# megvii-research/Far3D

Measured on AMD Instinct MI355X. Metric: samples/sec (7-cam frame) end-to-end @ VoV-99 640x960, higher is better.
Workload: dtype bf16x3; 1 GPU; BASELINE configs[1]: 7 cameras 3x640x960, VoV-99, A=1544 queries (644 learned + 644 adaptive + 256 propagated), 2312 self-attn keys, 6 decoder layers, streaming memory on, ego motion on; proposals=topk, fused_rows=True, parallelism=single GPU, weights=seeded random (far3d_amd.weights.init_state_dict, seed 0)

## Files before the change

### far3d_amd/csrc/conv_ws.hip

```cpp
#include "conv_ws.hpp"
#include "far3d_hip.h"

#ifdef FAR3D_PROFILING
std::atomic<int> g_ws_ablate{0};
extern "C" int far3d_conv_ws_set_ablate(int mask) { g_ws_ablate.store(mask); return 0; }
#endif

#define WS_CAPS_SINGLE(id, ...) case id: return Conv3x3WsShape<__VA_ARGS__>::caps;
#define WS_CAPS_GROUPED(id, ...)                                                   \
  case id: return Conv3x3WsShape<__VA_ARGS__>::caps | FAR3D_TILE_HAS_GROUP;        \
  case id + 100: return Conv3x3WsShape<__VA_ARGS__>::caps | FAR3D_TILE_GROUPED;
#define WS_CAPS_GROUPED_PLAIN(id, ...) WS_CAPS_GROUPED(id, __VA_ARGS__)
#define WS_CAPS(a, id, mark, ...) WS_CAPS_##mark(id, __VA_ARGS__)
#define WS_GROUP_SINGLE(id, ...)
#define WS_GROUP_GROUPED(id, ...) case id + 100: return launch_conv3x3_ws_grouped<true, __VA_ARGS__>(P, G, st);
#define WS_GROUP_GROUPED_PLAIN(id, ...) case id + 100: return launch_conv3x3_ws_grouped<false, __VA_ARGS__>(P, G, st);
#define WS_GROUP(a, id, mark, ...) WS_GROUP_##mark(id, __VA_ARGS__)
#define WS_LAUNCH(a, id, mark, ...) case id: return launch_conv3x3_ws<__VA_ARGS__>(P, st);

int far3d_ws_tile_caps(int tile) {
  switch (tile) {
    FAR3D_TILES_WS_CONV3(WS_CAPS, )
    FAR3D_TILES_WS_GEMM(TILE_CAPS, Gemm1x1WsShape)
    default: return -1;
  }
}

int far3d_conv_ws_launch(const IgemmParams& P, int tile, hipStream_t st) {
  switch (tile) {
    FAR3D_TILES_WS_CONV3(WS_LAUNCH, )
    default: break;
  }
  far3d_set_error("far3d_conv2d_nhwc: unknown wave-specialised tile %d", tile);
  return FAR3D_ERR_ARG;
}

extern "C" int far3d_ws_deal(int n_full, int n_light, int grid, int wg, int k) {
  if (n_full < 0 || n_light < 0 || grid < 1 || wg < 0 || wg >= grid) return -1;
  return ws_deal_item(n_full, n_light, grid, wg, k);
}

int far3d_gemm_ws_launch(const IgemmParams& P, int tile, hipStream_t st) {
  switch (tile) {
    FAR3D_TILES_WS_GEMM(TILE_LAUNCH, launch_gemm1x1_ws)
    default: break;
  }
  far3d_set_error("far3d_conv2d_nhwc: unknown wave-specialised GEMM tile %d", tile);
  return FAR3D_ERR_ARG;
}

static int far3d_conv_ws_grouped_launch(const IgemmParams& P, const WsGroup& G, int tile, hipStream_t st) {
  switch (tile) {
    FAR3D_TILES_WS_CONV3(WS_GROUP, )
    default: break;
  }
  far3d_set_error("far3d_conv2d_nhwc_grouped: unknown grouped tile %d", tile);
  return FAR3D_ERR_ARG;
}

extern "C" int far3d_conv2d_nhwc_grouped(const far3d_conv_problem* probs, int n, int tile, void* stream) {
  FAR3D_CHECK_ARG(probs && n >= 1 && n <= FAR3D_WS_GROUP_MAX, "far3d_conv2d_nhwc_grouped: %d problems (1..%d)", n, FAR3D_WS_GROUP_MAX);
  const int caps = far3d_ws_tile_caps(tile);
  FAR3D_CHECK_ARG(caps >= 0 && (caps & FAR3D_TILE_GROUPED), "far3d_conv2d_nhwc_grouped: tile %d is not a grouped tile (conv_tiles.hpp: 100 + a marked 4xx id)", tile);
  auto aligned = [](const void* p, long a) { return ((uintptr_t)p % a) == 0; };
  WsGroup G;
  memset(&G, 0, sizeof(G));
  G.n = n;
  const int Cin = probs[0].Cin;
  for (int i = 0; i < n; ++i) {
    const far3d_conv_problem& c = probs[i];
    FAR3D_CHECK_ARG(c.Cin == Cin, "far3d_conv2d_nhwc_grouped: problem %d has Cin %d, problem 0 has %d (one Cin per launch)", i, c.Cin, Cin);
    FAR3D_CHECK_ARG(c.x && c.w && c.y && c.N > 0 && c.H > 0 && c.W > 0 && c.Cout > 0 && Cin > 0 && Cin % 32 == 0 && c.Cout % 32 == 0 &&
                    c.act >= 0 && c.act <= 2 && c.ldx >= 2 * Cin && c.ldy >= 2 * c.Cout &&
                    aligned(c.x, 16) && aligned(c.y, 16) && c.ldx % 8 == 0 && c.ldy % 8 == 0 && c.x_img_stride % 8 == 0 && c.y_img_stride % 8 == 0 &&
                    (long)c.N * c.H * c.W < (1L << 31) - 4096 && (long)c.H * c.W * c.ldx * 2 < 0x7fffffffL,
                    "far3d_conv2d_nhwc_grouped: problem %d: needs pair-stored maps in and out, Cin and Cout multiples of 32, 16-byte aligned rows "
                    "(N=%d H=%d W=%d Cin=%d Cout=%d ldx=%d ldy=%d act=%d)", i, c.N, c.H, c.W, c.Cin, c.Cout, c.ldx, c.ldy, c.act);
    FAR3D_CHECK_ARG(!c.y2 || (c.y2_scale && c.y2_shift && aligned(c.y2, 16) && aligned(c.y2_scale, 16) && aligned(c.y2_shift, 16) &&
                              c.ldy2 >= c.Cout && c.ldy2 % 4 == 0 && c.y2_img_stride % 4 == 0),
                    "far3d_conv2d_nhwc_grouped: problem %d: the second output is fp32 with 16-byte aligned rows, scale and shift", i);
    WsProblem& q = G.p[i];
// ... 20 lines not shown
```

### far3d_amd/csrc/conv_ws.hpp

```cpp
#pragma once
#include "igemm_kernels.hpp"
#include <type_traits>

__device__ __forceinline__ __amdgpu_buffer_rsrc_t uniform_rsrc(const void* p, long nbytes) {
  const unsigned long long a = (unsigned long long)(uintptr_t)p;
  const unsigned lo = __builtin_amdgcn_readfirstlane((unsigned)a), hi = __builtin_amdgcn_readfirstlane((unsigned)(a >> 32));
  const int nb = __builtin_amdgcn_readfirstlane((int)(nbytes < 0x7fffffffL ? nbytes : 0x7fffffffL));
  return __builtin_amdgcn_make_buffer_rsrc((void*)(uintptr_t)(((unsigned long long)hi << 32) | lo), 0, nb, 0x00020000);
}

__device__ __forceinline__ void wait_vmcnt_dyn(int n) {
#define FAR3D_WVC(k) case k: wait_vmcnt<k>(); break;
  switch (n) {
    FAR3D_WVC(0) FAR3D_WVC(1) FAR3D_WVC(2) FAR3D_WVC(3) FAR3D_WVC(4) FAR3D_WVC(5) FAR3D_WVC(6) FAR3D_WVC(7) FAR3D_WVC(8)
    FAR3D_WVC(9) FAR3D_WVC(10) FAR3D_WVC(11) FAR3D_WVC(12) FAR3D_WVC(13) FAR3D_WVC(14) FAR3D_WVC(15) FAR3D_WVC(16)
    FAR3D_WVC(17) FAR3D_WVC(18) FAR3D_WVC(19) FAR3D_WVC(20) FAR3D_WVC(21) FAR3D_WVC(22) FAR3D_WVC(23) FAR3D_WVC(24)
    FAR3D_WVC(25) FAR3D_WVC(26) FAR3D_WVC(27) FAR3D_WVC(28) FAR3D_WVC(29) FAR3D_WVC(30) FAR3D_WVC(31) FAR3D_WVC(32)
    FAR3D_WVC(33) FAR3D_WVC(34) FAR3D_WVC(35) FAR3D_WVC(36) FAR3D_WVC(37) FAR3D_WVC(38) FAR3D_WVC(39) FAR3D_WVC(40)
    FAR3D_WVC(41) FAR3D_WVC(42) FAR3D_WVC(43) FAR3D_WVC(44) FAR3D_WVC(45) FAR3D_WVC(46) FAR3D_WVC(47)
    default: wait_vmcnt<48>(); break;
  }
#undef FAR3D_WVC
}

// ... 594 lines not shown
            const float4 bq = b4[q >> 1][q & 1];
            pacc[i][j][4 * q + 0] = acc[i][j][4 * q + 0] + bq.x; pacc[i][j][4 * q + 1] = acc[i][j][4 * q + 1] + bq.y;
            pacc[i][j][4 * q + 2] = acc[i][j][4 * q + 2] + bq.z; pacc[i][j][4 * q + 3] = acc[i][j][4 * q + 3] + bq.w;
          }
      }
      pd_n = n; pd_y0 = y0; pd_x0 = x0; pd_m0 = m0; pd_prob = prob;
    } else {
#pragma unroll
      for (int j = 0; j < WN; ++j)
#pragma unroll
        for (int i = 0; i < WM; ++i)
#pragma unroll
          for (int qp = 0; qp < 2; ++qp) {
            float4 b4[2];
            epi_bias(i, qp, m0, prob, b4);
            epi_slice(std::false_type{}, acc, i, j, qp, n, y0, x0, m0, prob, &b4);
          }
    }
#ifdef FAR3D_PROFILING
    if (pf_on) pf_epi += __builtin_amdgcn_s_memtime() - pf_e0;
#endif
  }
#ifdef FAR3D_PROFILING
  if (P.prof && t == 0) {
    P.prof[(long)blockIdx.x * 16 + 3] = (unsigned long long)__builtin_amdgcn_s_memtime();
    P.prof[(long)blockIdx.x * 16 + 7] = (unsigned long long)__builtin_amdgcn_s_memrealtime();
    P.prof[(long)blockIdx.x * 16 + 5] = (unsigned long long)total_steps;
    P.prof[(long)blockIdx.x * 16 + 8] = pf_wait; P.prof[(long)blockIdx.x * 16 + 9] = pf_body; P.prof[(long)blockIdx.x * 16 + 10] = pf_epi;
  }
#endif
#endif
}

template <int WGM, int WGN, int WM, int WN, int NP, int NSW, int GRP, bool SUMS>
__global__ __launch_bounds__(64 * (WGM * WGN + NP)) void gemm1x1_ws_kernel(IgemmParams P, int npt, int nct, int ablate) {
#if defined(__HIP_DEVICE_COMPILE__)
  constexpr int NWC = WGM * WGN;
  constexpr int BM = 32 * WGM * WM, BP = 32 * WGN * WN;
  constexpr int GA = BM / 16, GB = BP / 16, SLOTS = GA + GB;
  static_assert(SLOTS % NP == 0, "every producer issues the same number of pieces per step (counted vmcnt)");
  constexpr int SPW = SLOTS / NP;
  constexpr int SUB = (BM + BP) * 64, STAGE = 2 * SUB;
  static_assert(NSW % GRP == 0 && NSW / GRP >= 2, "ring = at least two hand-over groups");
  constexpr int NG = NSW / GRP;
  extern __shared__ __attribute__((aligned(1024))) unsigned char smem[];
  const int t = threadIdx.x, lane = t & 63, wv = __builtin_amdgcn_readfirstlane(t >> 6);
  constexpr int SUMB = NSW * STAGE;
  static_assert(SUMB + 4 * BM * 8 <= 163840, "LDS budget");
  [[maybe_unused]] long long* const lsum = reinterpret_cast<long long*>(smem + SUMB);
  constexpr bool do_sums = SUMS;
  if (do_sums) {
    for (int i = threadIdx.x; i < 4 * BM; i += 64 * (NWC + NP)) lsum[i] = 0;
    __syncthreads();
  }
  const int HoWo = P.Ho * P.Wo;
  const long Npix = (long)P.N * HoWo;
  const int nsteps = P.cin_pad / 32;
  const int Ktot = P.cin_pad * 2;
  const int xcd = (int)blockIdx.x & 7, slot0 = (int)blockIdx.x >> 3, dslot = (int)gridDim.x >> 3;
  const int vslots = ((npt - xcd + 7) >> 3) * nct;
  const int my_items = vslots > slot0 ? (vslots - slot0 + dslot - 1) / dslot : 0;
  const int total_steps = my_items * nsteps;
  const int total_groups = (total_steps + GRP - 1) / GRP;
  auto decode = [&](int k, int& p0, int& m0) __attribute__((always_inline)) {
    const int slot = slot0 + k * dslot;
    const int ct = slot % nct, pt = (slot / nct) * 8 + xcd;
    p0 = __builtin_amdgcn_readfirstlane(pt * BP); m0 = __builtin_amdgcn_readfirstlane(ct * BM);
  };

  if (wv >= NWC) {
    const int pw = wv - NWC;
    const int rg = lane >> 2, pc = lane & 3;
    const int lc = pc ^ ((rg >> 2) & 3);
    constexpr unsigned OOB = 0x80000000u;
    const long x_bytes = ((long)(P.N - 1) * P.x_img_stride + (long)HoWo * P.ldx) * 2;
    unsigned voff[SPW];
    int sdst[SPW];
    bool isw[SPW];
#pragma unroll
    for (int i = 0; i < SPW; ++i) {
      const int q = pw + NP * i;
      isw[i] = q < GA;
      const int g = isw[i] ? q : q - GA;
      sdst[i] = (isw[i] ? 0 : BM * 64) + g * 1024;
      voff[i] = isw[i] ? (unsigned)(((g * 16 + rg) * Ktot + lc * 8) * 2) : 0u;
    }
    const bf16_t* w_base = nullptr;
    long w_bytes = 0;
    int cur_tile = 0, cur_step = 0, cur_stage = 0, left = total_steps;
    auto set_tile = [&](int k) __attribute__((always_inline)) {
      int p0, m0;
      decode(k, p0, m0);
      w_base = reinterpret_cast<const bf16_t*>(P.w) + (long)m0 * Ktot;
      w_bytes = w_tile_bytes(BM, m0, P.Cout, Ktot);
#pragma unroll
      for (int i = 0; i < SPW; ++i) {
        if (!isw[i]) {
          const int g = pw + NP * i - GA;
          const long p = (long)p0 + g * 16 + rg;
          if (p < Npix) {
            int n, rem;
            pix_split(p, HoWo, n, rem);
            voff[i] = (unsigned)(((long)n * P.x_img_stride + (long)rem * P.ldx + lc * 8) * 2);
          } else {
            voff[i] = OOB;
          }
        }
      }
    };
    auto next = [&]() __attribute__((always_inline)) {
      if (!(ablate & 1)) {
        const __amdgpu_buffer_rsrc_t rs_w = uniform_rsrc(w_base, w_bytes);
        const __amdgpu_buffer_rsrc_t rs_x = uniform_rsrc(P.x, x_bytes);
        const int sbase = __builtin_amdgcn_readfirstlane(cur_stage * STAGE);
        const int kb = __builtin_amdgcn_readfirstlane(cur_step * 128);
#pragma unroll
        for (int i = 0; i < SPW; ++i) {
#pragma unroll
          for (int pl = 0; pl < 2; ++pl) {
            if (isw[i])
              __builtin_amdgcn_raw_ptr_buffer_load_lds(rs_w, (lds_void_t*)(smem + sbase + pl * SUB + sdst[i]), 16, voff[i], kb + pl * 64, 0, 0);
            else
              __builtin_amdgcn_raw_ptr_buffer_load_lds(rs_x, (lds_void_t*)(smem + sbase + pl * SUB + sdst[i]), 16, voff[i], kb + pl * 64, 0, 0);
          }
        }
      }
      --left;
      cur_stage = cur_stage == NSW - 1 ? 0 : cur_stage + 1;
      if (++cur_step == nsteps) { cur_step = 0; ++cur_tile; if (left > 0) set_tile(cur_tile); }
    };
    if (my_items > 0) set_tile(0);
#pragma unroll
    for (int i = 0; i < (NG - 1) * GRP; ++i)
      if (left > 0) next();
    for (int g = 0; g < total_groups; ++g) {
      int later = total_steps - (g + 1) * GRP;
      later = later < 0 ? 0 : (later > (NG - 2) * GRP ? (NG - 2) * GRP : later);
      if (ablate & 1) wait_vmcnt<0>(); else wait_vmcnt_dyn(later * SPW * 2);
      __builtin_amdgcn_s_barrier();
      asm volatile("" ::: "memory");
#pragma unroll
      for (int i = 0; i < GRP; ++i)
        if (left > 0) next();
    }
    if (do_sums) __builtin_amdgcn_s_barrier();
    return;
  }

  const int wm = wv / WGN, wn = wv % WGN, l31 = lane & 31, hi = lane >> 5;
  int aaddr[WM], baddr[WN];
#pragma unroll
  for (int i = 0; i < WM; ++i) {
    const int r = (wm * WM + i) * 32 + l31;
    aaddr[i] = r * 64 + ((hi ^ ((r >> 2) & 3)) << 4);
  }
#pragma unroll
  for (int j = 0; j < WN; ++j) {
    const int r = (wn * WN + j) * 32 + l31;
    baddr[j] = BM * 64 + r * 64 + ((hi ^ ((r >> 2) & 3)) << 4);
  }
  f32x16_t acc[WM][WN];
  u32x4_t fa[2][2][WM], fb[2][2][WN];
  auto load_a = [&](int set, int soff, int kk) __attribute__((always_inline)) {
    const int x32 = kk * 32;
#pragma unroll
    for (int pl = 0; pl < 2; ++pl)
#pragma unroll
      for (int i = 0; i < WM; ++i) fa[set][pl][i] = *reinterpret_cast<const u32x4_t*>(smem + pl * SUB + ((aaddr[i] ^ x32) + soff));
  };
  auto load_b = [&](int set, int soff, int kk) __attribute__((always_inline)) {
    const int x32 = kk * 32;
#pragma unroll
    for (int pl = 0; pl < 2; ++pl)
#pragma unroll
      for (int j = 0; j < WN; ++j) fb[set][pl][j] = *reinterpret_cast<const u32x4_t*>(smem + pl * SUB + ((baddr[j] ^ x32) + soff));
  };
  auto mma_term = [&](int set, int term) __attribute__((always_inline)) {
    const int pa = term == 0 ? 1 : 0, pb = term == 1 ? 1 : 0;
#pragma unroll
    for (int i = 0; i < WM; ++i)
#pragma unroll
      for (int j = 0; j < WN; ++j) mma<bf16_t>(acc[i][j], fa[set][pa][i], fb[set][pb][j]);
  };
  int soff = 0, gs = 0;
  [[maybe_unused]] int flush_tile = 0, gcount = 0;
  auto flush = [&](int T) __attribute__((always_inline)) {
    int fp0, fm0;
    decode(T, fp0, fm0);
    const int fcam0 = (int)((long)fp0 / P.sums_hw);
    long long* src = lsum + (T & 1) * 2 * BM;
    for (int i = wv * 64 + lane; i < 2 * BM; i += 64 * NWC) {
      const int sl = i / BM, chn = i - sl * BM, cam = fcam0 + sl;
      const long long v = src[i];
      if (v != 0) {
        src[i] = 0;
        if (cam < P.N && fm0 + chn < P.Cout)
          atomicAdd(reinterpret_cast<unsigned long long*>(P.chan_sums + (long)cam * P.Cout + fm0 + chn), (unsigned long long)v);
      }
    }
  };
  for (int k = 0; k < my_items; ++k) {
    int p0, m0;
    decode(k, p0, m0);
#pragma unroll
    for (int i = 0; i < WM; ++i)
#pragma unroll
      for (int j = 0; j < WN; ++j)
#pragma unroll
        for (int r = 0; r < 16; ++r) acc[i][j][r] = 0.f;
    for (int s = 0; s < nsteps; ++s) {
      const int stage = soff;
      if (gs == 0) {
        __builtin_amdgcn_s_waitcnt(0xc07f);
        __builtin_amdgcn_s_barrier();
        asm volatile("" ::: "memory");
        __builtin_amdgcn_sched_barrier(0);
        if constexpr (do_sums) {
          while (flush_tile < k && ((flush_tile + 1) * nsteps - 1) / GRP < gcount) { flush(flush_tile); ++flush_tile; }
          ++gcount;
        }
      }
      gs = gs == GRP - 1 ? 0 : gs + 1;
      if (ablate & 2) { soff = soff == (NSW - 1) * STAGE ? 0 : soff + STAGE; continue; }
      load_a(0, stage, 0); load_b(0, stage, 0);
      __builtin_amdgcn_sched_barrier(0);
      if (s > 0) { mma_term(1, 0); mma_term(1, 1); mma_term(1, 2); }
      __builtin_amdgcn_sched_barrier(0);
      load_a(1, stage, 1);
      __builtin_amdgcn_sched_barrier(0);
      mma_term(0, 0);
      __builtin_amdgcn_sched_barrier(0);
      load_b(1, stage, 1);
      __builtin_amdgcn_sched_barrier(0);
      mma_term(0, 1);
      mma_term(0, 2);
      __builtin_amdgcn_sched_barrier(0);
      soff = soff == (NSW - 1) * STAGE ? 0 : soff + STAGE;
    }
    if (!(ablate & 2)) { mma_term(1, 0); mma_term(1, 1); mma_term(1, 2); }
    __builtin_amdgcn_sched_barrier(0);

    {
      unsigned char* yb = reinterpret_cast<unsigned char*>(P.y);
      const int cam0 = do_sums ? (int)((long)p0 / P.sums_hw) : 0;
      const long bnd = (long)(cam0 + 1) * P.sums_hw;
      const bool two = do_sums && (long)p0 + BP > bnd;
      long pix_b[WN];
      bool okj[WN], secj[WN];
#pragma unroll
      for (int j = 0; j < WN; ++j) {
        const long p = (long)p0 + (wn * WN + j) * 32 + l31;
        okj[j] = p < Npix;
        secj[j] = p >= bnd;
        pix_b[j] = 0;
        if (okj[j]) {
          int n, rem;
          pix_split(p, HoWo, n, rem);
          pix_b[j] = ((long)n * P.y_img_stride + (long)rem * P.ldy) * 2;
        }
      }
      auto stored = [&](int i, int j, int q, int cb, uint2& h, uint2& l) __attribute__((always_inline)) {
        float4 b4 = make_float4(0.f, 0.f, 0.f, 0.f);
        if (P.bias) b4 = *reinterpret_cast<const float4*>(P.bias + cb + 8 * q + 4 * hi);
        float v[4];
#pragma unroll
        for (int e = 0; e < 4; ++e) v[e] = acc[i][j][4 * q + e];
        v[0] += b4.x; v[1] += b4.y; v[2] += b4.z; v[3] += b4.w;
        if (P.act == ACT_RELU) {
#pragma unroll
          for (int e = 0; e < 4; ++e) v[e] = fmaxf(v[e], 0.f);
        } else if (P.act == ACT_SWISH) {
#pragma unroll
          for (int e = 0; e < 4; ++e) v[e] = v[e] * (1.f / (1.f + expf(-v[e])));
        }
        split4f(v[0], v[1], v[2], v[3], h, l);
      };
      auto quantise = [&](const uint2& h, const uint2& l, int q, int (&qs)[16], float& mx) __attribute__((always_inline)) {
        const unsigned w4[4] = {h.x, h.y, l.x, l.y};
#pragma unroll
        for (int e = 0; e < 2; ++e) {
          const float h0 = __uint_as_float(w4[e] << 16), h1 = __uint_as_float(w4[e] & 0xffff0000u);
          const float l0 = __uint_as_float(w4[2 + e] << 16), l1 = __uint_as_float(w4[2 + e] & 0xffff0000u);
          mx = fmaxf(mx, fmaxf(fabsf(h0), fabsf(h1)));
          qs[4 * q + 2 * e] += __float2int_rn(h0 * (float)(1 << FAR3D_SUMS_FRAC_BITS)) + __float2int_rn(l0 * (float)(1 << FAR3D_SUMS_FRAC_BITS));
          qs[4 * q + 2 * e + 1] += __float2int_rn(h1 * (float)(1 << FAR3D_SUMS_FRAC_BITS)) + __float2int_rn(l1 * (float)(1 << FAR3D_SUMS_FRAC_BITS));
        }
      };
      auto half_sum = [&](int x) __attribute__((always_inline)) -> int {
        x += __builtin_amdgcn_update_dpp(0, x, 0x128, 0xf, 0xf, true);
        x += __builtin_amdgcn_update_dpp(0, x, 0x124, 0xf, 0xf, true);
        x += __builtin_amdgcn_update_dpp(0, x, 0x122, 0xf, 0xf, true);
        x += __builtin_amdgcn_update_dpp(0, x, 0x121, 0xf, 0xf, true);
        typedef unsigned u2_t __attribute__((ext_vector_type(2)));
        const u2_t r = __builtin_amdgcn_permlane16_swap((unsigned)x, (unsigned)x, false, false);
        const unsigned rx = r.x, ry = r.y;
        return (int)(rx + ry);
      };
      auto reduce_add = [&](const int (&qs)[16], float mx, int sl, int cb) __attribute__((always_inline)) {
        const bool wide = WN > 2 || __any(mx >= (float)(1 << (24 - FAR3D_SUMS_FRAC_BITS)));
        long long* dst = lsum + ((k & 1) * 2 + sl) * BM + (cb - m0) + 4 * hi;
#pragma unroll
        for (int r = 0; r < 16; ++r) {
          long long tot;
          if (!wide) {
            tot = (long long)half_sum(qs[r]);
          } else {
            const int lo16 = qs[r] & 0xffff, hi16 = qs[r] >> 16;
            tot = (long long)half_sum(hi16) * 65536ll + (long long)half_sum(lo16);
          }
          if (l31 == 0 && tot != 0) atomicAdd(reinterpret_cast<unsigned long long*>(dst + 8 * (r >> 2) + (r & 3)), (unsigned long long)tot);
        }
      };
      auto channel_block = [&](auto ic) __attribute__((always_inline)) {
        constexpr int i = decltype(ic)::value;
        const int cb = m0 + (wm * WM + i) * 32;
        if (cb >= P.Cout) return;
        int qs[16];
        float mx = 0.f;
#pragma unroll
        for (int r = 0; r < 16; ++r) qs[r] = 0;
#pragma unroll
        for (int j = 0; j < WN; ++j) {
#pragma unroll
          for (int qp = 0; qp < 2; ++qp) {
            uint2 h[2], l[2];
#pragma unroll
            for (int u = 0; u < 2; ++u) {
              stored(i, j, 2 * qp + u, cb, h[u], l[u]);
              if (do_sums && okj[j] && !secj[j]) quantise(h[u], l[u], 2 * qp + u, qs, mx);
            }
            u32x4_t oh, ol;
            {
              const auto sx = __builtin_amdgcn_permlane32_swap(h[0].x, h[1].x, false, false);
              const auto sy = __builtin_amdgcn_permlane32_swap(h[0].y, h[1].y, false, false);
              oh = u32x4_t{sx[0], sy[0], sx[1], sy[1]};
            }
            {
              const auto sx = __builtin_amdgcn_permlane32_swap(l[0].x, l[1].x, false, false);
              const auto sy = __builtin_amdgcn_permlane32_swap(l[0].y, l[1].y, false, false);
              ol = u32x4_t{sx[0], sy[0], sx[1], sy[1]};
            }
            if (okj[j]) {
              unsigned char* d = yb + pix_b[j] + (long)(cb >> 5) * 128 + (2 * qp + hi) * 16;
              *reinterpret_cast<u32x4_t*>(d) = oh;
              *reinterpret_cast<u32x4_t*>(d + 64) = ol;
            }
          }
        }
        if constexpr (do_sums) {
          auto exact_add = [&](int sl) __attribute__((always_inline)) {
            long long* dst = lsum + ((k & 1) * 2 + sl) * BM + (cb - m0) + 4 * hi;
#pragma unroll
            for (int q = 0; q < 4; ++q) {
              long long x[4] = {0, 0, 0, 0};
#pragma unroll
// ... 14 lines not shown
#pragma unroll
              for (int e = 0; e < 4; ++e) {
                const long long v = x[e];
                const long long tot = (long long)half_sum((int)(v & 0xffff)) + ((long long)half_sum((int)((v >> 16) & 0xffff)) << 16) +
                                      ((long long)half_sum((int)((v >> 32) & 0xffff)) << 32) + ((long long)half_sum((int)(v >> 48)) << 48);
                if (l31 == 0 && tot != 0) atomicAdd(reinterpret_cast<unsigned long long*>(dst + 8 * q + e), (unsigned long long)tot);
              }
            }
          };
          const bool huge = __any(mx >= 2048.f);
          if (huge) exact_add(0); else reduce_add(qs, mx, 0, cb);
          if (two) {
            float mx1 = 0.f;
#pragma unroll
            for (int r = 0; r < 16; ++r) qs[r] = 0;
#pragma unroll
            for (int j = 0; j < WN; ++j)
#pragma unroll
              for (int q = 0; q < 4; ++q) {
                uint2 h, l;
                stored(i, j, q, cb, h, l);
                if (okj[j] && secj[j]) quantise(h, l, q, qs, mx1);
              }
            if (__any(mx1 >= 2048.f)) exact_add(1); else reduce_add(qs, mx1, 1, cb);
          }
        }
      };
      static_assert(WM <= 4, "channel blocks per consumer");
      channel_block(std::integral_constant<int, 0>{});
      if constexpr (WM > 1) channel_block(std::integral_constant<int, 1>{});
      if constexpr (WM > 2) channel_block(std::integral_constant<int, 2>{});
      if constexpr (WM > 3) channel_block(std::integral_constant<int, 3>{});
    }
  }
  if constexpr (do_sums) {
    __builtin_amdgcn_s_waitcnt(0xc07f);
    __builtin_amdgcn_s_barrier();
    asm volatile("" ::: "memory");
    while (flush_tile < my_items) { flush(flush_tile); ++flush_tile; }
  }
#endif
}

static int ws_cu_count() {
  static std::atomic<int> n_cu{0};
  int cus = n_cu.load(std::memory_order_relaxed);
  if (cus == 0) {
    int dev = 0;
    if (hipGetDevice(&dev) != hipSuccess) dev = 0;
    if (hipDeviceGetAttribute(&cus, hipDeviceAttributeMultiprocessorCount, dev) != hipSuccess || cus <= 0) cus = 256;
    n_cu.store(cus, std::memory_order_relaxed);
  }
  return cus;
}
constexpr int ws_wg_per_cu(size_t lds, int threads) { return lds <= 81920 && threads <= 1024 ? 2 : 1; }

template <int WGM, int WGN, int WM, int WN, int NP, int NSW, int GRP>
struct Gemm1x1WsShape {
  static constexpr int BM = 32 * WGM * WM, BP = 32 * WGN * WN, THREADS = 64 * (WGM * WGN + NP);
  static constexpr size_t lds = (size_t)NSW * 2 * (BM + BP) * 64 + 4 * BM * 8;
  static constexpr int wg_per_cu = ws_wg_per_cu(lds, THREADS);
  static constexpr int caps = tile_caps(FAR3D_TILE_1X1, FAR3D_TILE_PAIR, BP, FAR3D_TILE_LDS_DMA | FAR3D_TILE_PERSISTENT | FAR3D_TILE_SUMS);
};

template <int WGM, int WGN, int WM, int WN, int NP, int NSW, int GRP>
static int launch_gemm1x1_ws(const IgemmParams& P, hipStream_t st) {
  using S = Gemm1x1WsShape<WGM, WGN, WM, WN, NP, NSW, GRP>;
  constexpr int BM = S::BM, BP = S::BP;
  constexpr size_t lds = S::lds;
  static_assert(lds <= 163840, "LDS budget");
  const long Npix = (long)P.N * P.Ho * P.Wo;
  const int npt = (int)((Npix + BP - 1) / BP), nct = (P.Cout + BM - 1) / BM;
  static std::atomic<unsigned long long> lds_ok_s{0};
  const long items = (long)((npt + 7) / 8 * 8) * nct;
  long grid = (long)ws_cu_count() * S::wg_per_cu;
  grid = (grid + 7) / 8 * 8;
  if (items < grid) grid = items;
  static std::atomic<unsigned long long> lds_ok{0};
  if constexpr (lds > 65536)
    if (const int rc = far3d_allow_lds(P.chan_sums ? reinterpret_cast<const void*>(&gemm1x1_ws_kernel<WGM, WGN, WM, WN, NP, NSW, GRP, true>)
                                                   : reinterpret_cast<const void*>(&gemm1x1_ws_kernel<WGM, WGN, WM, WN, NP, NSW, GRP, false>),
                                       (int)lds, P.chan_sums ? lds_ok_s : lds_ok, "far3d_conv2d_nhwc")) return rc;
  if (P.chan_sums) {
    if (P.sums_hw < BP || P.cin_pad / 32 < 2 * GRP) {
      far3d_set_error("far3d_conv2d_nhwc: channel sums on this wave-specialised GEMM tile need Ho*Wo (%d) >= %d pixels and Cin >= %d", P.sums_hw, BP, 64 * GRP);
      return FAR3D_ERR_ARG;
    }
    hipLaunchKernelGGL((gemm1x1_ws_kernel<WGM, WGN, WM, WN, NP, NSW, GRP, true>), dim3((unsigned)grid), dim3(S::THREADS), lds, st, P, npt, nct, FAR3D_WS_ABLATE_ARG);
  } else {
    hipLaunchKernelGGL((gemm1x1_ws_kernel<WGM, WGN, WM, WN, NP, NSW, GRP, false>), dim3((unsigned)grid), dim3(S::THREADS), lds, st, P, npt, nct, FAR3D_WS_ABLATE_ARG);
  }
  return 0;
}

template <int WGM, int WGN, int WM, int WN, int NP, bool PAIR, bool DBUF, int NSW = 3, bool FLAGS = false, int GRP = 1, bool DEFER = false>
struct Conv3x3WsShape {
  static constexpr int BM = 32 * WGM * WM, TH = WGN * WN, PLD = PAIR ? 2 : 1, THREADS = 64 * (WGM * WGN + NP);
  static constexpr int PG = (34 * (TH + 2) + 15) / 16;
  static constexpr size_t lds = (size_t)NSW * PLD * BM * 64 + (size_t)2 * PLD * PG * 1024 + (FLAGS ? 128 : 0);
  static constexpr int wg_per_cu = ws_wg_per_cu(lds, THREADS);
  static constexpr int caps = tile_caps(FAR3D_TILE_3X3, PAIR ? FAR3D_TILE_PAIR : FAR3D_TILE_BF16, 32 * TH, FAR3D_TILE_LDS_DMA | FAR3D_TILE_PERSISTENT);
};

template <bool DEFER_OK, int WGM, int WGN, int WM, int WN, int NP, bool PAIR, bool DBUF, int NSW = 3, bool FLAGS = false, int GRP = 1, bool DEFER = false, class GT>
static int launch_conv3x3_ws_items(const IgemmParams& P, hipStream_t st, int tiles_x, int tiles_y, int n_mt, int n_items, const GT& G, const char* who) {
  using S = Conv3x3WsShape<WGM, WGN, WM, WN, NP, PAIR, DBUF, NSW, FLAGS, GRP, DEFER>;
  static_assert(S::lds <= 163840, "LDS budget");
  const int resident = ws_cu_count() * S::wg_per_cu;
  const int grid = n_items < resident ? n_items : resident;
  static std::atomic<unsigned long long> lds_ok{0};
  if constexpr (S::lds > 65536)
    if (const int rc = far3d_allow_lds(reinterpret_cast<const void*>(&conv3x3_ws_kernel<WGM, WGN, WM, WN, NP, PAIR, DBUF, NSW, FLAGS, GRP, GT, DEFER && DEFER_OK>), (int)S::lds, lds_ok, who)) return rc;
  hipLaunchKernelGGL((conv3x3_ws_kernel<WGM, WGN, WM, WN, NP, PAIR, DBUF, NSW, FLAGS, GRP, GT, DEFER && DEFER_OK>), dim3((unsigned)grid), dim3(S::THREADS), S::lds, st, P, tiles_x, tiles_y,
                     n_mt, n_items, FAR3D_WS_ABLATE_ARG, G);
  return 0;
}

template <int WGM, int WGN, int WM, int WN, int NP, bool PAIR, bool DBUF, auto... MORE>
static int launch_conv3x3_ws(const IgemmParams& P, hipStream_t st) {
  using S = Conv3x3WsShape<WGM, WGN, WM, WN, NP, PAIR, DBUF, MORE...>;
  const int tiles_x = (P.Wo + 31) / 32, tiles_y = (P.Ho + S::TH - 1) / S::TH, n_mt = (P.Cout + S::BM - 1) / S::BM;
  return launch_conv3x3_ws_items<true, WGM, WGN, WM, WN, NP, PAIR, DBUF, MORE...>(P, st, tiles_x, tiles_y, n_mt, P.N * tiles_x * tiles_y * n_mt, WsSingle{}, "far3d_conv2d_nhwc");
}

// ... 21 lines not shown
```

### far3d_amd/lib.py

```python
import ctypes
import os

os.environ.setdefault("GPU_MAX_HW_QUEUES", "8")

import torch

_HERE = os.path.dirname(os.path.abspath(__file__))
LIB_PATH = os.path.join(_HERE, "libfar3d_hip.so")

c_int, c_float, c_void_p, c_char_p = ctypes.c_int, ctypes.c_float, ctypes.c_void_p, ctypes.c_char_p
c_long = ctypes.c_long
_p = c_void_p

SIGNATURES = {
    "far3d_last_error": (c_char_p, []),
    "far3d_abi_version": (c_int, []),
    "far3d_device_count": (c_int, []),
    "far3d_device_arch": (c_int, [c_int, c_char_p, c_int]),
    "far3d_msda_forward": (c_int, [_p, c_int, _p, _p, _p, _p, _p] + [c_int] * 7 + [_p]),
    "far3d_aggregate_forward": (c_int, [_p, c_int, _p, _p, _p, _p, _p, _p, _p, _p, c_int] + [c_int] * 7 +
                                [_p, _p, _p, c_float, c_float, c_int, c_int, c_int, _p, _p, c_int, _p, _p]),
    "far3d_aggregate_batched": (c_int, [_p, c_int, _p, _p, _p, _p, _p, _p, _p, c_int] + [c_int] * 8 +
                                [_p, _p, _p, c_float, c_float, c_int, c_int, _p]),
    "far3d_agg_operands": (c_int, [_p] * 8 + [c_int] * 6 + [_p, c_float, c_float, c_int, c_int, c_int, _p]),
    "far3d_camera_sum": (c_int, [_p, _p, c_int, c_int, c_int, c_int, _p]),
    "far3d_conv2d_nhwc": (c_int, [_p, c_int, _p, c_int, _p, _p, c_int] + [c_int] * 5 + [c_long] + [c_int] * 4 +
                          [c_long] + [c_int] * 5 + [_p, c_int, c_int, c_long, c_int, c_int] +
                          [_p, c_int, c_int, c_long, _p, _p, _p, c_int, _p]),
    "far3d_conv2d_nhwc_grouped": (c_int, [_p, c_int, c_int, _p]),
    "far3d_ws_deal": (c_int, [c_int] * 5),
    "far3d_conv_tile_caps": (c_int, [c_int] * 3),
    "far3d_attention_forward": (c_int, [_p, _p, _p, c_int, _p, c_int] + [c_int] * 8 + [c_float, _p, c_int, c_int, _p]),
    "far3d_attention_f32_variant": (c_int, [c_int]),
    "far3d_attention_streams": (c_int, [_p, _p, _p, c_int, _p, c_int] + [c_int] * 9 + [c_long] * 4 + [c_float, _p, c_int, c_int, _p]),
    "far3d_attention_batched": (c_int, [_p, _p, _p, c_int, _p, c_int] + [c_int] * 9 + [c_long] * 4 +
                                [c_float, _p, c_int, c_int, c_long, _p, _p]),
    "far3d_layernorm": (c_int, [_p, _p, _p, _p, c_int, c_int, c_int, c_int, c_float, c_int, _p, c_int, _p, c_int, c_int, _p, c_int, c_int, _p]),
    "far3d_layernorm_rows": (c_int, [_p, _p, _p, _p, c_int, c_int, c_int, c_int, c_float, c_int, _p, c_int, _p, c_int, c_int, _p, c_int, c_int, _p, _p]),
    "far3d_rowchain_attn_out": (c_int, [_p, c_int, _p, c_int, _p, c_int, _p, _p, _p, _p, _p, _p, c_int, _p, c_int, _p, c_int,
                                        _p, c_int, c_float, _p]),
    "far3d_rowchain_ffn": (c_int, [_p, c_int, _p, c_int, _p, c_int] + [_p] * 12 + [_p, c_int, _p, c_int, _p, c_int, c_int, c_float, _p]),
    "far3d_rowchain_qkv": (c_int, [_p, c_int, _p, c_int, _p, _p, _p, c_int, c_int, _p]),
    "far3d_rowchain_branches": (c_int, [_p, c_int] + [_p] * 10 + [c_int] + [_p] * 6 + [c_int, _p, c_int, _p, c_int, c_int, c_float, _p]),
    "far3d_ese_nhwc": (c_int, [_p, c_int, _p, _p, _p, _p, _p, c_int, c_int, c_int, c_int, c_long, c_int, c_long,
                               c_int, c_long, _p, _p]),
    "far3d_ese_fused_nhwc": (c_int, [_p, c_int, _p, _p, _p, _p, _p, _p, c_int, c_int, c_int, c_int, c_int, c_long, c_int, c_long, c_int, c_long,
                                     c_int, c_int, c_int, c_long, _p, _p]),
    "far3d_cam_embed_chain": (c_int, [_p] * 10 + [c_int, c_int, c_int, c_int, c_float, c_int, _p]),
    "far3d_groupnorm_nhwc": (c_int, [_p, c_int, _p, _p, _p, _p, c_int, c_int, c_int, c_int, c_float, c_int, _p]),
    "far3d_maxpool3x3s2_nhwc": (c_int, [_p, c_int, _p] + [c_int] * 7 + [c_long, _p]),
    "far3d_dwconv3x3_nhwc": (c_int, [_p, c_int, _p, _p, c_int, c_int, c_int, c_int, c_int, c_long, c_int, c_int, c_int, c_long, c_int, _p]),
    "far3d_dwconv3x3_act_nhwc": (c_int, [_p, c_int, _p, _p, _p, c_int, c_int, c_int, c_int, c_int, c_long, c_int, c_int, c_int, c_long,
                                         c_int, c_int, c_int, _p]),
    "far3d_dwsep_conv_nhwc": (c_int, [_p, c_int, _p, _p, c_int, _p, c_int, _p, c_int, _p, c_int, c_int, c_int, c_int, c_int, c_long,
                                      c_int, c_int, c_int, c_int, c_long, c_int, _p]),
    "far3d_stem_im2col": (c_int, [_p, _p, c_int, c_int, c_int, c_int, _p]),
    "far3d_stem_conv": (c_int, [_p, _p, _p, _p, c_int, c_int, c_int, c_int, c_long, c_int, _p]),
    "far3d_proposal_select": (c_int, [_p, _p, c_int, c_int, c_int, c_int, _p, _p, _p, _p, _p, _p, c_int, c_float, c_int, _p]),
    "far3d_proposal_gather": (c_int, [_p, c_int, c_int, c_int, _p, _p, _p, _p, c_int, _p, _p, c_int, c_int, c_int, c_int,
                                      c_float, c_float, c_int, _p, _p, c_int, c_int, _p, c_float, _p, _p, _p, _p, c_int, _p, _p, _p]),
    "far3d_proposal_gather_md": (c_int, [_p, c_int, c_int, c_int, _p, _p, _p, _p, c_int, _p, _p, c_int, c_int, c_int, c_int,
                                         c_float, c_float, c_int, _p, _p, c_int, c_int, _p, c_float, _p, _p, _p, _p, c_int,
                                         c_int, c_int, _p, _p, _p]),
# ... 66 lines not shown
```

### include/far3d_hip.h

```cpp
#ifndef FAR3D_HIP_H
#define FAR3D_HIP_H
#include <stdint.h>

#ifdef __cplusplus
extern "C" {
#endif

#define FAR3D_DT_F32 0
#define FAR3D_DT_BF16 1
#define FAR3D_DT_F32_BF16X3 2
#define FAR3D_DT_BF16_PAIR 3
#define FAR3D_SUMS_MAX_PARTS 32
#define FAR3D_SUMS_FRAC_BITS 18
#define FAR3D_SUMS_SCRATCH_FLOATS(N, C) ((long)(N) * (C) * (2 * FAR3D_SUMS_MAX_PARTS + 1))

#define FAR3D_OK 0
#define FAR3D_ERR_ARG (-1)
#define FAR3D_ERR_LAUNCH (-2)
#define FAR3D_ERR_UNSUPPORTED (-3)

const char* far3d_last_error(void);
int far3d_abi_version(void);
int far3d_device_count(void);
int far3d_device_arch(int dev, char* buf, int buflen);
// ... 41 lines not shown
  float* y2;
  const float* y2_scale;
  const float* y2_shift;
  long x_img_stride, y_img_stride, y2_img_stride;
  int N, H, W, Cin, Cout, ldx, ldy, ldy2;
  int act;
} far3d_conv_problem;
#define FAR3D_WS_GROUP_MAX 16

int far3d_conv2d_nhwc_grouped(const far3d_conv_problem* probs, int n, int tile, void* stream);

#define FAR3D_TILE_GEOM 3
#define FAR3D_TILE_ANY 0
#define FAR3D_TILE_1X1 1
#define FAR3D_TILE_3X3 2
#define FAR3D_TILE_3X3S2 3
#define FAR3D_TILE_STORE(caps) (((caps) >> 2) & 7)
#define FAR3D_TILE_BF16 0
#define FAR3D_TILE_PAIR 1
#define FAR3D_TILE_F32_SPLIT 2
#define FAR3D_TILE_F32 3
#define FAR3D_TILE_F32_BF16 4
#define FAR3D_TILE_HI_ONLY 32
#define FAR3D_TILE_PERSISTENT 64
#define FAR3D_TILE_HAS_GROUP 128
#define FAR3D_TILE_GROUPED 256
#define FAR3D_TILE_SUMS 512
#define FAR3D_TILE_LDS_DMA 1024
#define FAR3D_TILE_PIXELS(caps) ((caps) >> 16)
int far3d_conv_tile_caps(int tile, int x_dt, int w_dt);

int far3d_ws_deal(int n_full, int n_light, int grid, int wg, int k);

int far3d_attention_forward(const void* q, const void* k, const void* v, int dtype, void* out, int out_dt, int Aq, int Nk,
                            int heads, int head_dim, int ldq, int ldk, int ldv, int ldo, float scale,
                            const int32_t* hole_count, int hole_start, int hole_end, void* stream);

int far3d_attention_f32_variant(int variant);

int far3d_attention_streams(const void* q, const void* k, const void* v, int dtype, void* out, int out_dt, int B, int Aq, int Nk,
                            int heads, int head_dim, int ldq, int ldk, int ldv, int ldo, long bsq, long bsk, long bsv, long bso,
                            float scale, const int32_t* hole_count, int hole_start, int hole_end, void* stream);

int far3d_attention_batched(const void* q, const void* k, const void* v, int dtype, void* out, int out_dt, int B, int Aq, int Nk,
                            int heads, int head_dim, int ldq, int ldk, int ldv, int ldo, long bsq, long bsk, long bsv, long bso,
                            float scale, const void* attn_mask, int mask_kind, int ldm, long mask_bstride,
                            const uint8_t* key_padding, void* stream);

int far3d_layernorm(const float* x, const float* gamma, const float* beta, float* y, int rows, int C, int ldx,
                    int ldy, float eps, int act, const float* add, int lda, void* y2, int ldy2, int y2_dt, void* yb, int ldyb,
                    int yb_dt, void* stream);
int far3d_layernorm_rows(const float* x, const float* gamma, const float* beta, float* y, int rows, int C, int ldx,
                         int ldy, float eps, int act, const float* add, int lda, void* y2, int ldy2, int y2_dt, void* yb, int ldyb,
                         int yb_dt, const int32_t* out_rows, void* stream);

int far3d_rowchain_attn_out(const void* att, int ld_att, const float* x, int ldx, const float* qpos, int ldq,
                            const void* w_out, const float* b_out, const float* g0, const float* be0,
                            const void* w_wl, const float* b_wl, int n_wl, float* x1, int ldx1, float* ul, int ldu,
                            const int32_t* ul_rows, int M, float eps, void* stream);

int far3d_rowchain_ffn(const void* agg, int ld_agg, const float* x1, int ldx1, const float* qpos, int ldq,
                       const void* w_o, const float* b_o, const float* g1, const float* be1,
                       const void* w_1, const float* b_1, const void* w_2, const float* b_2,
                       const float* g2, const float* be2, const void* w_qkv, const float* b_qkv,
                       float* out, int ldo, void* qkv, int ldqkv, void* xop, int ldxop, int M, float eps, void* stream);

// ... 149 lines not shown
```

Measured before the change: 76.01 samples/s.

## Split tail work items of the persistent 1x1 GEMM into halves or quarters

The persistent wave-specialised 1x1 GEMM kernel now deals its last partial round of output tiles differently. When the leftover tile count is small relative to the grid, each leftover tile is split into two pixel halves or four pixel/channel quarters, so more workgroups share the final wave instead of a few doing whole tiles. This adds templated reduced-size MMA loops, adjusted load offsets and epilogue bounds, plus host-side deal/resident query functions and profiling hooks. The risks are extra code size, register pressure from the added instantiations, and correctness in the index remapping.

```diff
diff --git a/far3d_amd/csrc/conv_ws.hip b/far3d_amd/csrc/conv_ws.hip
--- a/far3d_amd/csrc/conv_ws.hip
+++ b/far3d_amd/csrc/conv_ws.hip
@@ -47,6 +47,22 @@
   }
   far3d_set_error("far3d_conv2d_nhwc: unknown wave-specialised GEMM tile %d", tile);
   return FAR3D_ERR_ARG;
+}
+
+#define WS_GEMM_DEAL(a, id, ...) case id: return gemm1x1_ws_deal<__VA_ARGS__>(npix, cout, grid, wg, k, out6);
+#define WS_GEMM_RESIDENT(a, id, ...) case id: return (ws_cu_count() * Gemm1x1WsShape<__VA_ARGS__>::wg_per_cu + 7) / 8 * 8;
+extern "C" int far3d_gemm_ws_deal(int tile, long long npix, int cout, int grid, int wg, int k, int* out6) {
+  if (npix < 1 || npix >= (1LL << 31) - 4096 || cout < 1 || grid < 8 || grid % 8 || wg < 0 || wg >= grid || !out6) return -1;
+  switch (tile) {
+    FAR3D_TILES_WS_GEMM(WS_GEMM_DEAL, )
+    default: return -1;
+  }
+}
+extern "C" int far3d_gemm_ws_resident(int tile) {
+  switch (tile) {
+    FAR3D_TILES_WS_GEMM(WS_GEMM_RESIDENT, )
+    default: return -1;
+  }
 }
 
 static int far3d_conv_ws_grouped_launch(const IgemmParams& P, const WsGroup& G, int tile, hipStream_t st) {
diff --git a/far3d_amd/csrc/conv_ws.hpp b/far3d_amd/csrc/conv_ws.hpp
--- a/far3d_amd/csrc/conv_ws.hpp
+++ b/far3d_amd/csrc/conv_ws.hpp
@@ -650,8 +650,30 @@
 #endif
 }
 
+struct GemmWsTail { int q, r8, parts; };
+__host__ __device__ inline GemmWsTail gemm_ws_tail(long padded_items, int grid, int max_parts) {
+  GemmWsTail t;
+  t.q = (int)(padded_items / grid);
+  const int R = (int)(padded_items - (long)t.q * grid);
+  t.r8 = R >> 3;
+  t.parts = R > 0 && max_parts >= 4 && 4 * R <= grid ? 4 : (R > 0 && max_parts >= 2 && 2 * R <= grid ? 2 : 1);
+  return t;
+}
+struct GemmWsMine { int nfull, n, sub_slot, sub; };
+__host__ __device__ inline GemmWsMine gemm_ws_mine(const GemmWsTail& t, int npt, int nct, int grid, int b) {
+  const int xcd = b & 7, slot0 = b >> 3, dslot = grid >> 3, lg = t.parts >> 1;
+  const int vslots = ((npt - xcd + 7) >> 3) * nct;
+  const int valid = vslots > slot0 ? (vslots - slot0 + dslot - 1) / dslot : 0;
+  GemmWsMine m;
+  m.nfull = valid < t.q ? valid : t.q;
+  m.sub_slot = t.q * dslot + (slot0 >> lg);
+  m.sub = t.parts > 1 ? (slot0 & (t.parts - 1)) : -1;
+  m.n = m.nfull + (slot0 < (t.r8 << lg) && m.sub_slot < vslots ? 1 : 0);
+  return m;
+}
+
 template <int WGM, int WGN, int WM, int WN, int NP, int NSW, int GRP, bool SUMS>
-__global__ __launch_bounds__(64 * (WGM * WGN + NP)) void gemm1x1_ws_kernel(IgemmParams P, int npt, int nct, int ablate) {
+__global__ __launch_bounds__(64 * (WGM * WGN + NP)) void gemm1x1_ws_kernel(IgemmParams P, int npt, int nct, GemmWsTail tail, int ablate) {
 #if defined(__HIP_DEVICE_COMPILE__)
   constexpr int NWC = WGM * WGN;
   constexpr int BM = 32 * WGM * WM, BP = 32 * WGN * WN;
@@ -676,15 +698,29 @@
   const int nsteps = P.cin_pad / 32;
   const int Ktot = P.cin_pad * 2;
   const int xcd = (int)blockIdx.x & 7, slot0 = (int)blockIdx.x >> 3, dslot = (int)gridDim.x >> 3;
-  const int vslots = ((npt - xcd + 7) >> 3) * nct;
-  const int my_items = vslots > slot0 ? (vslots - slot0 + dslot - 1) / dslot : 0;
+  const GemmWsMine mine = gemm_ws_mine(tail, npt, nct, (int)gridDim.x, (int)blockIdx.x);
+  const int my_items = mine.n;
+  constexpr bool HALVES = WN >= 2, QUARTERS = WN >= 2 && WM >= 2;
+  const int sub_k = HALVES && mine.sub >= 0 ? mine.nfull : 0x7fffffff;
+  [[maybe_unused]] const int sub_h = mine.sub & 1;
+  [[maybe_unused]] const bool sub_q = QUARTERS && tail.parts == 4;
+  [[maybe_unused]] const int sub_c = sub_q ? (mine.sub >> 1) & 1 : 0;
   const int total_steps = my_items * nsteps;
   const int total_groups = (total_steps + GRP - 1) / GRP;
   auto decode = [&](int k, int& p0, int& m0) __attribute__((always_inline)) {
-    const int slot = slot0 + k * dslot;
+    const int slot = k < mine.nfull ? slot0 + k * dslot : mine.sub_slot;
     const int ct = slot % nct, pt = (slot / nct) * 8 + xcd;
     p0 = __builtin_amdgcn_readfirstlane(pt * BP); m0 = __builtin_amdgcn_readfirstlane(ct * BM);
   };
+#ifdef FAR3D_PROFILING
+  if (P.prof && t == 0) {
+    P.prof[(long)blockIdx.x * 16 + 6] = (unsigned long long)__builtin_amdgcn_s_memrealtime();
+    P.prof[(long)blockIdx.x * 16 + 1] = (unsigned long long)__builtin_amdgcn_s_memtime();
+    P.prof[(long)blockIdx.x * 16 + 4] = (unsigned long long)my_items;
+  }
+  unsigned long long pf_epi = 0;
+  const bool pf_on = P.prof != nullptr && wv == 0;
+#endif
 
   if (wv >= NWC) {
     const int pw = wv - NWC;
@@ -711,12 +747,29 @@
       decode(k, p0, m0);
       w_base = reinterpret_cast<const bf16_t*>(P.w) + (long)m0 * Ktot;
       w_bytes = w_tile_bytes(BM, m0, P.Cout, Ktot);
+      const bool sub = HALVES && k == sub_k;
 #pragma unroll
       for (int i = 0; i < SPW; ++i) {
-        if (!isw[i]) {
-          const int g = pw + NP * i - GA;
+        if (isw[i]) {
+          if constexpr (QUARTERS) {
+            if (sub && sub_q) {
+              const int g = pw + NP * i, st = g >> 1, wi = st % WM;
+              const int row = sub_c * (BM / 2) + ((st / WM) * (WM / 2) + wi) * 32 + (g & 1) * 16 + rg;
+              voff[i] = wi < WM / 2 ? (unsigned)((row * Ktot + lc * 8) * 2) : OOB;
+            }
+          }
+        } else {
+          int g = pw + NP * i - GA;
+          bool present = true;
+          if constexpr (HALVES) {
+            if (sub) {
+              const int st = g >> 1, wj = st % WN;
+              present = wj < WN / 2;
+              g = sub_h * (GB / 2) + (((st / WN) * (WN / 2) + wj) << 1) + (g & 1);
+            }
+          }
           const long p = (long)p0 + g * 16 + rg;
-          if (p < Npix) {
+          if (present && p < Npix) {
             int n, rem;
             pix_split(p, HoWo, n, rem);
             voff[i] = (unsigned)(((long)n * P.x_img_stride + (long)rem * P.ldx + lc * 8) * 2);
@@ -779,26 +832,26 @@
   }
   f32x16_t acc[WM][WN];
   u32x4_t fa[2][2][WM], fb[2][2][WN];
-  auto load_a = [&](int set, int soff, int kk) __attribute__((always_inline)) {
+  auto load_a = [&](auto mi, int set, int soff, int kk) __attribute__((always_inline)) {
     const int x32 = kk * 32;
 #pragma unroll
     for (int pl = 0; pl < 2; ++pl)
 #pragma unroll
-      for (int i = 0; i < WM; ++i) fa[set][pl][i] = *reinterpret_cast<const u32x4_t*>(smem + pl * SUB + ((aaddr[i] ^ x32) + soff));
+      for (int i = 0; i < decltype(mi)::value; ++i) fa[set][pl][i] = *reinterpret_cast<const u32x4_t*>(smem + pl * SUB + ((aaddr[i] ^ x32) + soff));
   };
-  auto load_b = [&](int set, int soff, int kk) __attribute__((always_inline)) {
+  auto load_b = [&](auto nj, int set, int soff, int kk) __attribute__((always_inline)) {
     const int x32 = kk * 32;
 #pragma unroll
     for (int pl = 0; pl < 2; ++pl)
 #pragma unroll
-      for (int j = 0; j < WN; ++j) fb[set][pl][j] = *reinterpret_cast<const u32x4_t*>(smem + pl * SUB + ((baddr[j] ^ x32) + soff));
+      for (int j = 0; j < decltype(nj)::value; ++j) fb[set][pl][j] = *reinterpret_cast<const u32x4_t*>(smem + pl * SUB + ((baddr[j] ^ x32) + soff));
   };
-  auto mma_term = [&](int set, int term) __attribute__((always_inline)) {
+  auto mma_term = [&](auto mi, auto nj, int set, int term) __attribute__((always_inline)) {
     const int pa = term == 0 ? 1 : 0, pb = term == 1 ? 1 : 0;
 #pragma unroll
-    for (int i = 0; i < WM; ++i)
-#pragma unroll
-      for (int j = 0; j < WN; ++j) mma<bf16_t>(acc[i][j], fa[set][pa][i], fb[set][pb][j]);
+    for (int i = 0; i < decltype(mi)::value; ++i)
+#pragma unroll
+      for (int j = 0; j < decltype(nj)::value; ++j) mma<bf16_t>(acc[i][j], fa[set][pa][i], fb[set][pb][j]);
   };
   int soff = 0, gs = 0;
   [[maybe_unused]] int flush_tile = 0, gcount = 0;
@@ -826,38 +879,53 @@
       for (int j = 0; j < WN; ++j)
 #pragma unroll
         for (int r = 0; r < 16; ++r) acc[i][j][r] = 0.f;
-    for (int s = 0; s < nsteps; ++s) {
-      const int stage = soff;
-      if (gs == 0) {
-        __builtin_amdgcn_s_waitcnt(0xc07f);
-        __builtin_amdgcn_s_barrier();
-        asm volatile("" ::: "memory");
+    auto run_steps = [&](auto mi, auto nj) __attribute__((always_inline)) {
+      for (int s = 0; s < nsteps; ++s) {
+        const int stage = soff;
+        if (gs == 0) {
+          __builtin_amdgcn_s_waitcnt(0xc07f);
+          __builtin_amdgcn_s_barrier();
+          asm volatile("" ::: "memory");
+          __builtin_amdgcn_sched_barrier(0);
+          if constexpr (do_sums) {
+            while (flush_tile < k && ((flush_tile + 1) * nsteps - 1) / GRP < gcount) { flush(flush_tile); ++flush_tile; }
+            ++gcount;
+          }
+        }
+        gs = gs == GRP - 1 ? 0 : gs + 1;
+        if (ablate & 2) { soff = soff == (NSW - 1) * STAGE ? 0 : soff + STAGE; continue; }
+        load_a(mi, 0, stage, 0); load_b(nj, 0, stage, 0);
         __builtin_amdgcn_sched_barrier(0);
-        if constexpr (do_sums) {
-          while (flush_tile < k && ((flush_tile + 1) * nsteps - 1) / GRP < gcount) { flush(flush_tile); ++flush_tile; }
-          ++gcount;
-        }
-      }
-      gs = gs == GRP - 1 ? 0 : gs + 1;
-      if (ablate & 2) { soff = soff == (NSW - 1) * STAGE ? 0 : soff + STAGE; continue; }
-      load_a(0, stage, 0); load_b(0, stage, 0);
+        if (s > 0) { mma_term(mi, nj, 1, 0); mma_term(mi, nj, 1, 1); mma_term(mi, nj, 1, 2); }
+        __builtin_amdgcn_sched_barrier(0);
+        load_a(mi, 1, stage, 1);
+        __builtin_amdgcn_sched_barrier(0);
+        mma_term(mi, nj, 0, 0);
+        __builtin_amdgcn_sched_barrier(0);
+        load_b(nj, 1, stage, 1);
+        __builtin_amdgcn_sched_barrier(0);
+        mma_term(mi, nj, 0, 1);
+        mma_term(mi, nj, 0, 2);
+        __builtin_amdgcn_sched_barrier(0);
+        soff = soff == (NSW - 1) * STAGE ? 0 : soff + STAGE;
+      }
+      if (!(ablate & 2)) { mma_term(mi, nj, 1, 0); mma_term(mi, nj, 1, 1); mma_term(mi, nj, 1, 2); }
       __builtin_amdgcn_sched_barrier(0);
-      if (s > 0) { mma_term(1, 0); mma_term(1, 1); mma_term(1, 2); }
-      __builtin_amdgcn_sched_barrier(0);
-      load_a(1, stage, 1);
-      __builtin_amdgcn_sched_barrier(0);
-      mma_term(0, 0);
-      __builtin_amdgcn_sched_barrier(0);
-      load_b(1, stage, 1);
-      __builtin_amdgcn_sched_barrier(0);
-      mma_term(0, 1);
-      mma_term(0, 2);
-      __builtin_amdgcn_sched_barrier(0);
-      soff = soff == (NSW - 1) * STAGE ? 0 : soff + STAGE;
-    }
-    if (!(ablate & 2)) { mma_term(1, 0); mma_term(1, 1); mma_term(1, 2); }
-    __builtin_amdgcn_sched_barrier(0);
-
+    };
+    const bool sub = HALVES && k == sub_k;
+    if constexpr (HALVES) {
+      if (!sub) run_steps(std::integral_constant<int, WM>{}, std::integral_constant<int, WN>{});
+      else if (!sub_q) run_steps(std::integral_constant<int, WM>{}, std::integral_constant<int, WN / 2>{});
+      else if constexpr (QUARTERS) run_steps(std::integral_constant<int, WM / 2>{}, std::integral_constant<int, WN / 2>{});
+    } else {
+      run_steps(std::integral_constant<int, WM>{}, std::integral_constant<int, WN>{});
+    }
+    const int mi_n = sub && sub_q ? WM / 2 : WM, nj_n = sub ? WN / 2 : WN;
+
+#ifdef FAR3D_PROFILING
+    unsigned long long pf_e0 = 0;
+    if (pf_on) pf_e0 = __builtin_amdgcn_s_memtime();
+#endif
     {
       unsigned char* yb = reinterpret_cast<unsigned char*>(P.y);
       const int cam0 = do_sums ? (int)((long)p0 / P.sums_hw) : 0;
@@ -867,8 +935,9 @@
       bool okj[WN], secj[WN];
 #pragma unroll
       for (int j = 0; j < WN; ++j) {
-        const long p = (long)p0 + (wn * WN + j) * 32 + l31;
-        okj[j] = p < Npix;
+        const int px = sub ? sub_h * (BP / 2) + (wn * (WN / 2) + j) * 32 : (wn * WN + j) * 32;
+        const long p = (long)p0 + px + l31;
+        okj[j] = p < Npix && j < nj_n;
         secj[j] = p >= bnd;
         pix_b[j] = 0;
         if (okj[j]) {
@@ -931,7 +1000,8 @@
       };
       auto channel_block = [&](auto ic) __attribute__((always_inline)) {
         constexpr int i = decltype(ic)::value;
-        const int cb = m0 + (wm * WM + i) * 32;
+        if (i >= mi_n) return;
+        const int cb = m0 + (sub && sub_q ? sub_c * (BM / 2) + (wm * (WM / 2) + i) * 32 : (wm * WM + i) * 32);
         if (cb >= P.Cout) return;
         int qs[16];
         float mx = 0.f;
@@ -939,6 +1009,7 @@
         for (int r = 0; r < 16; ++r) qs[r] = 0;
 #pragma unroll
         for (int j = 0; j < WN; ++j) {
+          if (j >= nj_n) continue;
 #pragma unroll
           for (int qp = 0; qp < 2; ++qp) {
             uint2 h[2], l[2];
@@ -1019,7 +1090,18 @@
       if constexpr (WM > 2) channel_block(std::integral_constant<int, 2>{});
       if constexpr (WM > 3) channel_block(std::integral_constant<int, 3>{});
     }
-  }
+#ifdef FAR3D_PROFILING
+    if (pf_on) pf_epi += __builtin_amdgcn_s_memtime() - pf_e0;
+#endif
+  }
+#ifdef FAR3D_PROFILING
+  if (P.prof && t == 0) {
+    P.prof[(long)blockIdx.x * 16 + 3] = (unsigned long long)__builtin_amdgcn_s_memtime();
+    P.prof[(long)blockIdx.x * 16 + 7] = (unsigned long long)__builtin_amdgcn_s_memrealtime();
+    P.prof[(long)blockIdx.x * 16 + 5] = (unsigned long long)total_steps;
+    P.prof[(long)blockIdx.x * 16 + 10] = pf_epi;
+  }
+#endif
   if constexpr (do_sums) {
     __builtin_amdgcn_s_waitcnt(0xc07f);
     __builtin_amdgcn_s_barrier();
@@ -1047,6 +1129,7 @@
   static constexpr int BM = 32 * WGM * WM, BP = 32 * WGN * WN, THREADS = 64 * (WGM * WGN + NP);
   static constexpr size_t lds = (size_t)NSW * 2 * (BM + BP) * 64 + 4 * BM * 8;
   static constexpr int wg_per_cu = ws_wg_per_cu(lds, THREADS);
+  static constexpr int max_parts = WN >= 2 ? (WM >= 2 ? 4 : 2) : 1;
   static constexpr int caps = tile_caps(FAR3D_TILE_1X1, FAR3D_TILE_PAIR, BP, FAR3D_TILE_LDS_DMA | FAR3D_TILE_PERSISTENT | FAR3D_TILE_SUMS);
 };
 
@@ -1063,6 +1146,7 @@
   long grid = (long)ws_cu_count() * S::wg_per_cu;
   grid = (grid + 7) / 8 * 8;
   if (items < grid) grid = items;
+  const GemmWsTail tail = gemm_ws_tail(items, (int)grid, (FAR3D_WS_ABLATE_ARG & 32) ? 1 : S::max_parts);
   static std::atomic<unsigned long long> lds_ok{0};
   if constexpr (lds > 65536)
     if (const int rc = far3d_allow_lds(P.chan_sums ? reinterpret_cast<const void*>(&gemm1x1_ws_kernel<WGM, WGN, WM, WN, NP, NSW, GRP, true>)
@@ -1073,10 +1157,30 @@
       far3d_set_error("far3d_conv2d_nhwc: channel sums on this wave-specialised GEMM tile need Ho*Wo (%d) >= %d pixels and Cin >= %d", P.sums_hw, BP, 64 * GRP);
       return FAR3D_ERR_ARG;
     }
-    hipLaunchKernelGGL((gemm1x1_ws_kernel<WGM, WGN, WM, WN, NP, NSW, GRP, true>), dim3((unsigned)grid), dim3(S::THREADS), lds, st, P, npt, nct, FAR3D_WS_ABLATE_ARG);
+    hipLaunchKernelGGL((gemm1x1_ws_kernel<WGM, WGN, WM, WN, NP, NSW, GRP, true>), dim3((unsigned)grid), dim3(S::THREADS), lds, st, P, npt, nct, tail, FAR3D_WS_ABLATE_ARG);
   } else {
-    hipLaunchKernelGGL((gemm1x1_ws_kernel<WGM, WGN, WM, WN, NP, NSW, GRP, false>), dim3((unsigned)grid), dim3(S::THREADS), lds, st, P, npt, nct, FAR3D_WS_ABLATE_ARG);
-  }
+    hipLaunchKernelGGL((gemm1x1_ws_kernel<WGM, WGN, WM, WN, NP, NSW, GRP, false>), dim3((unsigned)grid), dim3(S::THREADS), lds, st, P, npt, nct, tail, FAR3D_WS_ABLATE_ARG);
+  }
+  return 0;
+}
+
+template <int WGM, int WGN, int WM, int WN, int NP, int NSW, int GRP>
+static int gemm1x1_ws_deal(long npix, int cout, int grid, int wg, int k, int* out) {
+  using S = Gemm1x1WsShape<WGM, WGN, WM, WN, NP, NSW, GRP>;
+  const int npt = (int)((npix + S::BP - 1) / S::BP), nct = (cout + S::BM - 1) / S::BM;
+  const GemmWsTail tail = gemm_ws_tail((long)((npt + 7) / 8 * 8) * nct, grid, S::max_parts);
+  const GemmWsMine m = gemm_ws_mine(tail, npt, nct, grid, wg);
+  if (k < 0 || k >= m.n) return -1;
+  const bool sub = k >= m.nfull && m.sub >= 0;
+  const int slot = k < m.nfull ? (wg >> 3) + k * (grid >> 3) : m.sub_slot;
+  const int ct = slot % nct, pt = (slot / nct) * 8 + (wg & 7);
+  long p0 = (long)pt * S::BP, p1 = p0 + S::BP;
+  int c0 = ct * S::BM, c1 = c0 + S::BM;
+  if (sub) { p0 += (m.sub & 1) * (S::BP / 2); p1 = p0 + S::BP / 2; }
+  if (sub && tail.parts == 4) { c0 += ((m.sub >> 1) & 1) * (S::BM / 2); c1 = c0 + S::BM / 2; }
+  out[0] = sub ? tail.parts : 1; out[1] = ct;
+  out[2] = (int)(p0 < npix ? p0 : npix); out[3] = (int)(p1 < npix ? p1 : npix);
+  out[4] = c0 < cout ? c0 : cout; out[5] = c1 < cout ? c1 : cout;
   return 0;
 }
 
diff --git a/far3d_amd/lib.py b/far3d_amd/lib.py
--- a/far3d_amd/lib.py
+++ b/far3d_amd/lib.py
@@ -29,6 +29,8 @@
                           [_p, c_int, c_int, c_long, _p, _p, _p, c_int, _p]),
     "far3d_conv2d_nhwc_grouped": (c_int, [_p, c_int, c_int, _p]),
     "far3d_ws_deal": (c_int, [c_int] * 5),
+    "far3d_gemm_ws_deal": (c_int, [c_int, ctypes.c_longlong, c_int, c_int, c_int, c_int, _p]),
+    "far3d_gemm_ws_resident": (c_int, [c_int]),
     "far3d_conv_tile_caps": (c_int, [c_int] * 3),
     "far3d_attention_forward": (c_int, [_p, _p, _p, c_int, _p, c_int] + [c_int] * 8 + [c_float, _p, c_int, c_int, _p]),
     "far3d_attention_f32_variant": (c_int, [c_int]),
diff --git a/include/far3d_hip.h b/include/far3d_hip.h
--- a/include/far3d_hip.h
+++ b/include/far3d_hip.h
@@ -97,6 +97,9 @@
 
 int far3d_ws_deal(int n_full, int n_light, int grid, int wg, int k);
 
+int far3d_gemm_ws_deal(int tile, long long npix, int cout, int grid, int wg, int k, int* out6);
+int far3d_gemm_ws_resident(int tile);
+
 int far3d_attention_forward(const void* q, const void* k, const void* v, int dtype, void* out, int out_dt, int Aq, int Nk,
                             int heads, int head_dim, int ldq, int ldk, int ldv, int ldo, float scale,
                             const int32_t* hole_count, int hole_start, int hole_end, void* stream);
```

New measurement: 75.99 samples/s. About the same (-0.0%).
